# roboyu/Kimera-Multi

Measured on AMD Instinct MI355X. Metric: dpgo edges*iters/sec (+ LC candidates verified/sec in 'lcd'), higher is better.
Workload: dtype f64

## Files before the change

kimera-multi_amd/csrc/pgo.hip:

```cpp
#include <hip/hip_runtime.h>
#include <hip/hip_ext.h>
#include <rccl/rccl.h>
#include <dlfcn.h>

#include <algorithm>
#include <chrono>
#include <thread>
#include <cmath>
#include <cstdio>
#include <cstdlib>
#include <cstring>
#include <limits>
#include <numeric>
#include <string>
#include <vector>

#include "common.h"

#ifndef KMX_HESS_PROBE
#define KMX_HESS_PROBE 0
#endif

namespace {

constexpr int WAVES = 4;
constexpr int BLOCK = 64 * WAVES;
constexpr int NPART = 4;
constexpr int RED_BYTES = 8 * NPART * WAVES + 16;

enum Phase { PH_IDLE = 0, PH_START = 1, PH_TCG = 2, PH_STEP = 3 };
// ... 35 lines not shown
__device__ __forceinline__ Gnc load_gnc(const Gnc* p) {
  Gnc s;
  s.inner = p->inner; s.updates = p->updates; s.fired = p->fired; s.rounds = p->rounds;
  s.mu = p->mu; s.pad[0] = s.pad[1] = s.pad[2] = 0.0;
  return s;
}
__device__ __forceinline__ void store_gnc(Gnc* p, const Gnc& s) {
  p->inner = s.inner; p->updates = s.updates; p->fired = s.fired; p->rounds = s.rounds; p->mu = s.mu;
}

struct HostStatus {
  unsigned long long word;
};
__device__ __forceinline__ void post_status(HostStatus* hs, int l, unsigned long long seq, bool running) {
  __hip_atomic_store(&hs[l].word, (seq << 1) | (running ? 1ull : 0ull), __ATOMIC_RELAXED, __HIP_MEMORY_SCOPE_SYSTEM);
}

struct Params {
  int tcg_max, rtr_iters, use_precond, robust;
  double kappa, theta, Delta0, Delta_max, accept_rho, gn_tol, shift, barc, mu_step, rel_tol;
  int gnc_on, inner_iters, max_updates, n_ext;
  int rgd;
  double rgd_step;
  int early_stop;
};

struct alignas(16) TileDesc {
  int robot, p0, k0, np_n;
  int rt0, rt1;
  int pad0, pad1;
};

struct Dev {
  int ntiles, L, nloc, npub;
  int gt0, gnt;
  const TileDesc* tile;
  const int* rtile0;
  const int* inc_ptr;
  double* rec;
  const int* rec_o;
  double* ekappa;
  double* etau;
  double* ew;
  const int2* eipos;
  double *X, *Xt, *g, *r, *z, *hd, *S, *Pinv, *hD, *pub;
  double* hDS;
  double* dh;
// ... 61 lines not shown
  return s;
}

template <int R>
__device__ __forceinline__ double gsum(double x, int base) {
  double s = 0.0;
#pragma unroll
  for (int k = 0; k < R; ++k) s += __shfl(x, base + k, 64);
  return s;
}

__device__ __forceinline__ void load4(const double* p, double v[4]) {
  const double2* q = reinterpret_cast<const double2*>(p);
  double2 a = q[0], b = q[1];
  v[0] = a.x; v[1] = a.y; v[2] = b.x; v[3] = b.y;
}
__device__ __forceinline__ void store4(double* p, const double v[4]) {
  double2* q = reinterpret_cast<double2*>(p);
  q[0] = make_double2(v[0], v[1]);
  q[1] = make_double2(v[2], v[3]);
}

constexpr int SYM4 = 10;
__device__ __forceinline__ void load_sym4(const double* p, double M[16]) {
  const double2* p2 = reinterpret_cast<const double2*>(p);
  const double2 a = p2[0], b = p2[1], c = p2[2], e = p2[3], f = p2[4];
  M[0] = a.x; M[1] = M[4] = a.y; M[2] = M[8] = b.x; M[3] = M[12] = b.y;
  M[5] = c.x; M[6] = M[9] = c.y; M[7] = M[13] = e.x;
  M[10] = e.y; M[11] = M[14] = f.x;
  M[15] = f.y;
}
__device__ __forceinline__ void load_sym3(const double* p, double S[9]) {
  S[0] = p[0]; S[1] = S[3] = p[1]; S[2] = S[6] = p[2];
  S[4] = p[3]; S[5] = S[7] = p[4];
  S[8] = p[5];
}

__device__ __forceinline__ void lds_barrier() { asm volatile("s_waitcnt lgkmcnt(0)\n\ts_barrier" ::: "memory"); }

struct Edge {
  double R[9], t[3], wk, wt;
};

__device__ __forceinline__ int2 unpack_int2(double v) {
  const long long b = __double_as_longlong(v);
  return make_int2((int)(b & 0xffffffffll), (int)(b >> 32));
}

template <int RW>
struct Rec {
  static constexpr int Q = RW / 2;
  static constexpr int GS = RW == 10 ? 8 : 16;
  static constexpr int WK = RW == 10 ? 6 : 12;
  __device__ static __forceinline__ void load(const Dev& d, size_t k, double2 q[Q]) {
    if constexpr (RW == 10) {
      const double2* p2 = reinterpret_cast<const double2*>(d.rec + (size_t)GS * k);
      const double2 a0 = p2[0], a1 = p2[1], a2 = p2[2], a3 = p2[3];
      const unsigned raw = (unsigned)d.rec_o[k];
      const int other = (int)(raw << 3) >> 3;
      const unsigned big = raw >> 29;
      const double qa = a0.x, qb = a0.y, qc = a1.x;
      const double ql = sqrt(1.0 - (qa * qa + qb * qb + qc * qc));
      const double w = big == 0 ? ql : qa, x = big == 0 ? qa : (big == 1 ? ql : qb);
      const double y = big <= 1 ? qb : (big == 2 ? ql : qc), z = big == 3 ? ql : qc;
      q[0] = make_double2(w, x);
      q[1] = make_double2(y, z);
      q[2] = make_double2(a1.y, a2.x);
      q[3] = make_double2(a2.y, a3.x);
      const double wt = a3.y;
      const long long bits = (long long)(unsigned)other | (std::signbit(wt) ? (1ll << 63) : 0ll);
      q[4] = make_double2(std::fabs(wt), __longlong_as_double(bits));
    } else {
      const double2* q2 = reinterpret_cast<const double2*>(d.rec + (size_t)GS * k);
#pragma unroll
      for (int i = 0; i < Q; ++i) q[i] = q2[i];
    }
  }
  __device__ static __forceinline__ double wt_word(double wt, bool tail) {
    return (RW == 10 && tail) ? -wt : wt;
  }
  __device__ static __forceinline__ void edge(const double2 q[Q], Edge& E) {
    if constexpr (RW == 10) {
      const double w = q[0].x, x = q[0].y, y = q[1].x, z = q[1].y;
      const double xx = x * x, yy = y * y, zz = z * z, xy = x * y, xz = x * z, yz = y * z;
      const double wx = w * x, wy = w * y, wz = w * z;
      E.R[0] = 1.0 - 2.0 * (yy + zz); E.R[1] = 2.0 * (xy - wz); E.R[2] = 2.0 * (xz + wy);
      E.R[3] = 2.0 * (xy + wz); E.R[4] = 1.0 - 2.0 * (xx + zz); E.R[5] = 2.0 * (yz - wx);
      E.R[6] = 2.0 * (xz - wy); E.R[7] = 2.0 * (yz + wx); E.R[8] = 1.0 - 2.0 * (xx + yy);
      E.t[0] = q[2].x; E.t[1] = q[2].y; E.t[2] = q[3].x;
      E.wk = q[3].y;
      E.wt = q[4].x;
    } else {
      E.R[0] = q[0].x; E.R[1] = q[0].y; E.R[2] = q[1].x; E.R[3] = q[1].y; E.R[4] = q[2].x;
      E.R[5] = q[2].y; E.R[6] = q[3].x; E.R[7] = q[3].y; E.R[8] = q[4].x;
      E.t[0] = q[4].y; E.t[1] = q[5].x; E.t[2] = q[5].y;
      E.wk = q[6].x;
      E.wt = q[6].y;
    }
  }
// ... 191 lines not shown
  static constexpr int ptr_off = x_off + TP * R * 32;
  static constexpr int red_off = ptr_off + ((TP + 1) * 4 + 15) / 16 * 16;
  static constexpr int bytes = red_off + 8 * NPART * W + 16;
};
template <int R, int W = WAVES>
struct SmemC {
  static constexpr int TP = W * (64 / R);
  static constexpr int x_off = 0;
  static constexpr int ptr_off = TP * R * 32;
  static constexpr int red_off = ptr_off + ((TP + 1) * 4 + 15) / 16 * 16;
  static constexpr int bytes = red_off + 8 * NPART * W + 16;
};
constexpr int SCR_BYTES = BLOCK * 6 * 8;
struct SmemU {
  static constexpr int red_off = SCR_BYTES;
  static constexpr int bytes = red_off + RED_BYTES;
};
static_assert(SCR_BYTES <= SmemH<3>::ptr_off && SCR_BYTES <= SmemH<8>::ptr_off, "scratch");
static_assert(SCR_BYTES <= SmemHG<3>::x_off, "scratch");

struct NoPre {
  __device__ bool operator()() const { return true; }
};
template <int R, int RW, bool REC_FIRST, typename Src, typename Pre, bool DIAG = true, int W = WAVES>
__device__ __forceinline__ bool hinc_gather_src(const Dev& d, const Lane& L, Src& src, double acc[4], char* smem,
                                                Pre&& pre) {
  using SM = SmemH<R, W>;
  using RC = Rec<RW>;
  constexpr int CH = SM::CH;
  double* Cs = reinterpret_cast<double*>(smem + SM::c_off);
  int* sptr = reinterpret_cast<int*>(smem + SM::ptr_off);
  const int tid = threadIdx.x;
  const int p0 = L.p0, np = L.np, K0 = L.k0, n = L.n;
  const int pl = L.pose - p0;
  const int lt = min(tid, CH - 1);
  acc[0] = acc[1] = acc[2] = acc[3] = 0.0;
  auto ld = [&](int c0, double2* q) { RC::load(d, (size_t)(K0 + max(min(c0 + lt, n - 1), 0)), q); };
  double2 q[RC::Q];
  if constexpr (REC_FIRST) ld(0, q);
  if (tid <= np) sptr[tid] = d.inc_ptr[p0 + tid] - K0;
  if constexpr (!REC_FIRST) ld(0, q);
  __syncthreads();
  if (!pre()) return false;
  for (int c0 = 0; c0 < n; c0 += CH) {
    Edge E;
    RC::edge(q, E);
    const int2 in = RC::inc(q);
    const int o = in.x;
    const bool tail = (in.y >> 31) & 1;
    double2 vr[2 * R];
    src.nbr(o, vr);
    if (tid < CH && c0 + tid < n) {
      const double wk = (o >= 0) ? E.wk : 0.0, wt = (o >= 0) ? E.wt : 0.0;
#pragma unroll
      for (int a = 0; a < R; ++a) {
        const double v0 = vr[2 * a].x, v1 = vr[2 * a].y, v2 = vr[2 * a + 1].x, v3 = vr[2 * a + 1].y;
        double h[4];
        if (tail) {
#pragma unroll
          for (int c = 0; c < 3; ++c)
            h[c] = -(wk * (v0 * E.R[c * 3 + 0] + v1 * E.R[c * 3 + 1] + v2 * E.R[c * 3 + 2]) + wt * v3 * E.t[c]);
          h[3] = -(wt * v3);
        } else {
#pragma unroll
          for (int c = 0; c < 3; ++c) h[c] = -(wk * (v0 * E.R[0 * 3 + c] + v1 * E.R[1 * 3 + c] + v2 * E.R[2 * 3 + c]));
          h[3] = -(wt * (v3 + (v0 * E.t[0] + v1 * E.t[1] + v2 * E.t[2])));
        }
        store4(Cs + (tid * R + a) * 4, h);
      }
    }
    asm volatile("" ::: "memory");
    ld(c0 + CH, q);
    lds_barrier();
    if (L.valid) {
      const int j0 = max(sptr[pl], c0) - c0, j1 = min(sptr[pl + 1], c0 + CH) - c0;
#pragma unroll 4
      for (int j = j0; j < j1; ++j) {
        double h[4];
        load4(Cs + (j * R + L.a) * 4, h);
        acc[0] += h[0]; acc[1] += h[1]; acc[2] += h[2]; acc[3] += h[3];
      }
    }
    lds_barrier();
  }
  if (DIAG && L.valid) {
    double vs[4];
    double D[16];
    src.own(L.pose, L.a, vs);
#if KMX_HESS_PROBE & 2
    for (int c = 0; c < 16; ++c) D[c] = (c % 5 == 0) ? 1.0 : 0.0;
#else
    load_sym4(d.hD + SYM4 * (size_t)L.pose, D);
#endif
#pragma unroll
    for (int c = 0; c < 4; ++c)
      acc[c] += vs[0] * D[4 * c] + vs[1] * D[4 * c + 1] + vs[2] * D[4 * c + 2] + vs[3] * D[4 * c + 3];
  }
  return true;
}

template <int R>
struct PlainRows {
  const double* V;
  __device__ __forceinline__ void nbr(int o, double2 vr[2 * R]) const {
    const double2* b2 = reinterpret_cast<const double2*>(V + (size_t)max(o, 0) * 4 * R);
#if KMX_HESS_PROBE & 1
#pragma unroll
    for (int i = 0; i < 2 * R; ++i) vr[i] = make_double2(1e-3 * i, 1e-3);
    (void)b2;
#else
#pragma unroll
    for (int i = 0; i < 2 * R; ++i) vr[i] = b2[i];
#endif
  }
  __device__ __forceinline__ void own(int pose, int a, double vs[4]) {
#if KMX_HESS_PROBE & 2
    for (int c = 0; c < 4; ++c) vs[c] = 1e-3 * c;
#else
    load4(V + (size_t)pose * 4 * R + 4 * a, vs);
#endif
  }
};
template <int R, int RW, bool REC_FIRST = false, bool DIAG = true, typename Pre = NoPre>
__device__ __forceinline__ bool hinc_gather(const Dev& d, const Lane& L, const double* V, double acc[4],
                                            char* smem, Pre&& pre = Pre{}) {
  PlainRows<R> src{V};
  return hinc_gather_src<R, RW, REC_FIRST, PlainRows<R>, Pre&, DIAG, WAVES>(d, L, src, acc, smem, pre);
}

template <int R, int RW, int W = WAVES>
__device__ __forceinline__ void hinc_grad(const Dev& d, const Lane& L, const double* V, const double* pub,
                                          double acc[4], double* cost, char* smem) {
  using SM = SmemHG<R, W>;
  using RC = Rec<RW>;
  constexpr int CH = SM::CH;
  double* Cs = reinterpret_cast<double*>(smem + SM::c_off);
  double2* xs = reinterpret_cast<double2*>(smem + SM::x_off);
  int* sptr = reinterpret_cast<int*>(smem + SM::ptr_off);
  const int tid = threadIdx.x;
  const int p0 = L.p0, np = L.np, K0 = L.k0, n = L.n;
  const int pl = L.pose - p0;
  const int lt = min(tid, CH - 1);
  acc[0] = acc[1] = acc[2] = acc[3] = 0.0;
  double csum = 0.0;
  auto ld = [&](int c0, double2* q) { RC::load(d, (size_t)(K0 + max(min(c0 + lt, n - 1), 0)), q); };
  double2 q[RC::Q];
  ld(0, q);
  if (tid <= np) sptr[tid] = d.inc_ptr[p0 + tid] - K0;
  {
    const double2* v2 = reinterpret_cast<const double2*>(V + (size_t)p0 * 4 * R);
// ... 612 lines not shown
    }
    vals[0] = m;
    vals[1] = ch;
  }
  double* lds = reinterpret_cast<double*>(smem);
#pragma unroll
  for (int s = 0; s < 2; ++s) {
    const double w = wave_sum(vals[s]);
    if ((threadIdx.x & 63) == 0) lds[s * WAVES + (threadIdx.x >> 6)] = w;
  }
  __syncthreads();
  if (threadIdx.x == 0) {
#pragma unroll
    for (int s = 0; s < 2; ++s) {
      double t = 0.0;
#pragma unroll
      for (int w = 0; w < WAVES; ++w) t += lds[s * WAVES + w];
      d.part[(size_t)L.tile * NPART + 2 + s] = t;
    }
  }
}

template <int R, int RW, int RM>
__device__ __forceinline__ void body_hess(const Dev& d, int first_launch, int slot, HostStatus* hs,
                                          unsigned long long seq, char* smem) {
  const Lane L = lane_map<R>(d);
  int tcg_iter;
  double beta;
  double y[4] = {0, 0, 0, 0}, zs[4] = {0, 0, 0, 0}, H[4];
  const size_t o = (size_t)L.pose * 4 * R + 4 * L.a;
  if constexpr (RM == RM_CONSUMER) {
    __shared__ Ctl cs;
    __shared__ double rl[NPART * WAVES];
    const Ctl& c0 = d.ctl[L.l];
    const bool writer = L.tile == L.rt0;
    if (writer && threadIdx.x < (int)(sizeof(Ctl) / 8))
      reinterpret_cast<double*>(&cs)[threadIdx.x] = reinterpret_cast<const double*>(&c0)[threadIdx.x];
    const bool grad = (first_launch & 1) != 0;
    const bool upd = !grad;
    RobotSum<2> rs;
    RobotSum<3> rg;
    if (upd) rs.issue(d.part_u, 2, L.rt0, L.rt1);
    if (grad) rg.issue(d.part, NPART, L.rt0, L.rt1);
    const int ph0 = c0.phase;
    const bool active = ph0 == (grad ? PH_START : PH_TCG);
    auto idle = [&]() {
      if (writer && threadIdx.x == 0) {
        d.ctl2[L.l] = c0;
        if (hs) post_status(hs, L.l, seq, false);
      }
    };
    if (!active && (!d.p.early_stop || (first_launch & 2))) {
      idle();
      return;
    }
    UpdStep u{0, 0, 0.0};
    auto decide = [&]() {
      if (!active) {
        idle();
        return false;
      }
      double tot[NPART] = {0.0, 0.0, 0.0, 0.0};
      if (upd) rs.finish(d.part_u, 2, rl, tot);
      if (grad) rg.finish(d.part, NPART, rl, tot);
      if (upd) u = upd_step(c0.mode, c0.r_stop, c0.lin_stop, c0.z_r, c0.tcg_iter, tot[0], tot[1], d.p);
      if (grad) u.done = sqrt(tot[1]) < d.p.gn_tol ? 1 : 0;
      if (writer && threadIdx.x == 0) {
        if (upd || grad) control_on(cs, d, L.l, grad ? RED_GRAD : RED_UPDATE, tot, R, true);
        d.ctl2[L.l] = cs;
        if (hs) post_status(hs, L.l, seq, cs.phase == PH_TCG);
      }
      return !u.done;
    };
    bool go;
    if (d.p.early_stop) {
      go = hinc_gather<R, RW, false, false>(d, L, d.z, H, smem, decide);
    } else {
      hinc_gather<R, RW, false, false>(d, L, d.z, H, smem);
      go = decide();
    }
    if (!go) return;
    tcg_iter = grad ? 0 : c0.tcg_iter;
    beta = u.beta;
  } else {
    const Ctl& c = d.ctl[L.l];
    const int ph = c.phase;
    tcg_iter = c.tcg_iter;
    beta = c.beta;
    if ((first_launch & 2) && ph != PH_TCG) return;
    if (!hinc_gather<R, RW, true, false>(d, L, d.z, H, smem, [&]() { return ph == PH_TCG; })) return;
  }
  const bool first = (tcg_iter == 0) || (KMX_HESS_PROBE & 4);
  asm volatile("" ::: "memory");
  const int dhn = d.dhn;
  double dold[4] = {0, 0, 0, 0}, hold[4] = {0, 0, 0, 0};
  if (L.valid) {
    double Dg[16];
#if KMX_HESS_PROBE & 2
    for (int k = 0; k < 4; ++k) zs[k] = 1e-3 * k;
    for (int c = 0; c < 16; ++c) Dg[c] = (c % 5 == 0) ? 1.0 : 0.0;
#else
    load4(d.z + o, zs);
    load_sym4(d.hDS + SYM4 * (size_t)L.pose, Dg);
#endif
    if (!first) {
      load4(d.dh + (size_t)((tcg_iter - 1) % dhn) * d.vec + o, dold);
      load4(d.hd + o, hold);
    }
#pragma unroll
    for (int c = 0; c < 4; ++c)
      H[c] += zs[0] * Dg[4 * c] + zs[1] * Dg[4 * c + 1] + zs[2] * Dg[4 * c + 2] + zs[3] * Dg[4 * c + 3];
  }
  double hz[4];
#pragma unroll
  for (int k = 0; k < 4; ++k) hz[k] = H[k];
  (void)y;
  double v = 0.0;
  double dl[4] = {0, 0, 0, 0}, hdl[4] = {0, 0, 0, 0};
  if (L.valid) {
    if (first) {
#pragma unroll
      for (int k = 0; k < 4; ++k) { dl[k] = -zs[k]; hdl[k] = -hz[k]; }
    } else {
#pragma unroll
      for (int k = 0; k < 4; ++k) {
        dl[k] = -zs[k] + beta * dold[k];
        hdl[k] = -hz[k] + beta * hold[k];
      }
      if (tcg_iter >= dhn && tcg_iter % dhn == 0) {
        double et[4] = {0, 0, 0, 0};
        if (tcg_iter > dhn) load4(d.eta + o, et);
// ... 507 lines not shown
    if (threadIdx.x == 0 && writer) {
      control_on(cs, d, L.l, RED_COST, tot, R, true);
      cs.phase = PH_STEP;
      d.ctl[L.l] = cs;
    }
  } else {
    commit = d.ctl[L.l].commit != 0;
  }
  if (!commit || !L.valid) return;
  const size_t o = (size_t)L.pose * 4 * R + 4 * L.a;
  double v[4];
  load4(d.Xt + o, v);
  store4(d.X + o, v);
  if (!final) return;
  const int s = d.pose_slot[L.pose];
  if (s >= 0) store4(d.pub + (size_t)s * 4 * R + 4 * L.a, v);
}

template <int R, int RW, int RM>
__global__ __launch_bounds__(BLOCK, LB<R>::w) void k_grad(Dev d, int gated) {
  KMX_SMEM;
  body_grad<R, RW, RM>(d, gated, smem);
}
template <int R, int RW, int RM>
__global__ __launch_bounds__(BLOCK, LB<R>::w) void k_hess(Dev d, int first, int slot, HostStatus* hs,
                                                          unsigned long long seq) {
  KMX_SMEM;
  body_hess<R, RW, RM>(d, first, slot, hs, seq, smem);
}
template <int R, int RM>
__global__ __launch_bounds__(BLOCK) void k_update(Dev d, HostStatus* hs, unsigned long long seq, int slot) {
  KMX_SMEM;
  body_update<R, RM>(d, hs, seq, slot, smem);
}
template <int R, int RW>
__global__ __launch_bounds__(BLOCK, (R <= 5 ? 3 : 2)) void k_step(Dev d, const Ctl* cin, Ctl* cout, int jl, int slot,
                                                                  HostStatus* hs, unsigned long long seq) {
  KMX_SMEM;
  body_step<R, RW>(d, cin, cout, jl, slot, hs, seq, smem);
}
template <int R>
__global__ __launch_bounds__(BLOCK) void k_retract(Dev d, int fold, const Ctl* src) {
  KMX_SMEM;
  body_retract<R>(d, fold, src, smem);
}
template <int R, int RW, int RM>
__global__ __launch_bounds__(BLOCK, LB<R>::w) void k_cost(Dev d, const Ctl* src) {
  KMX_SMEM;
  body_cost<R, RW, RM>(d, src, smem);
}
template <int R>
// ... 456 lines not shown
  int *d_xs_rseg = nullptr, *d_xr_rseg = nullptr;
  double *d_xsbuf = nullptr, *d_xrbuf = nullptr;
  long long xn_send = 0, xn_recv = 0;
  std::vector<long long> xs_cnt, xr_cnt, xs_off, xr_off;
  int blind_left = 0;
  static constexpr int BLIND_SLACK = 2, BLIND_WINDOW = 8;
  static constexpr int MAX_GROUPS = 4;
  struct Group {
    int l0 = 0, l1 = 0;
    int t0 = 0, nt = 0;
    int blind_left = 0;
  };
  int groups_req = 2;
  std::vector<Group> grp;
  int grm = 2;
  int grm_forced = -1;
  static constexpr int GROUP_CONSUMER_MAX_TILES = 384;
  hipStream_t gstream[MAX_GROUPS - 1] = {nullptr, nullptr, nullptr};
  hipEvent_t ev_fork = nullptr, ev_join[MAX_GROUPS - 1] = {nullptr, nullptr, nullptr};
  bool hess_gate = true;
  int rm = RM_LAUNCH;
  int rm_forced = -1;
  int early_stop = 1;
  static constexpr int RM_CONSUMER_MAX_POSES = 80000;
  bool poll_timeout = false;
  bool timing = false;
  int* d_hv_launch = nullptr;
  std::vector<hipEvent_t> ev_pool;
  size_t ev_used = 0;
  double *d_accV = nullptr, *d_accY = nullptr;
  double acc_gamma = 0.0;
  int acc_k = 0;
  bool acc_ready = false, acc_started = false;
};

namespace {

void rot_to_quat(const double* R, double* q) {
  const double tr = R[0] + R[4] + R[8];
  double w, x, y, z;
  if (tr > 0.0) {
    const double s = 2.0 * std::sqrt(tr + 1.0);
    w = 0.25 * s; x = (R[7] - R[5]) / s; y = (R[2] - R[6]) / s; z = (R[3] - R[1]) / s;
  } else if (R[0] > R[4] && R[0] > R[8]) {
    const double s = 2.0 * std::sqrt(1.0 + R[0] - R[4] - R[8]);
    w = (R[7] - R[5]) / s; x = 0.25 * s; y = (R[1] + R[3]) / s; z = (R[2] + R[6]) / s;
// ... 119 lines not shown

void sync_params(kmx_pgo* h) {
  Params& p = h->dv.p;
  p.tcg_max = h->P.tcg_max_iterations;
  p.rtr_iters = h->P.rtr_iterations;
  p.use_precond = h->P.use_preconditioner;
  p.robust = h->P.robust_cost == KMX_COST_GNC_TLS ? 1 : 0;
  p.kappa = h->P.tcg_kappa;
  p.theta = h->P.tcg_theta;
  p.Delta0 = h->P.rtr_initial_radius;
  p.Delta_max = h->P.rtr_max_radius;
  p.accept_rho = h->P.rtr_accept_rho;
  p.gn_tol = h->P.gradnorm_tol;
  p.shift = h->P.precond_shift;
  p.barc = h->P.gnc_barc;
  p.mu_step = h->P.gnc_mu_step;
  p.rel_tol = h->gnc_rel_tol;
  p.gnc_on = h->gnc_on;
  p.inner_iters = h->gnc_inner_iters;
  p.max_updates = h->gnc_max_updates;
  p.n_ext = h->n_ext;
  p.rgd = h->P.method == KMX_METHOD_RGD ? 1 : 0;
  p.rgd_step = h->P.rgd_stepsize;
  p.early_stop = h->early_stop;
  h->dv.ext = h->d_ext;
}

void enqueue_publish(kmx_pgo* h) {
  const int ps = 4 * h->P.r;
  const long long tot = h->n_owned * ps;
  if (tot == 0) return;
  hipLaunchKernelGGL(k_publish, dim3((unsigned)((tot / 2 + 255) / 256)), dim3(256), 0, h->stream, h->d_vec,
                     h->d_pub + (size_t)h->first_owned * ps, h->d_pub_src + h->first_owned, (int)h->n_owned, ps);
}

template <int RW>
void enqueue_precond_t(kmx_pgo* h, int gated) {
  const int blocks = std::max(1, std::min(gated ? 256 : 1024, (h->nloc + 127) / 128));
  hipLaunchKernelGGL(k_precond<RW>, dim3(blocks), dim3(128), 0, h->stream, h->dv, gated);
}
void enqueue_precond(kmx_pgo* h, int gated) {
  if (h->rw == 10) enqueue_precond_t<10>(h, gated);
  else enqueue_precond_t<16>(h, gated);
}

bool enqueue_begin(kmx_pgo* h, const unsigned char* d_active, int mode, bool defer = false,
                   hipEvent_t done = nullptr) {
// ... 61 lines not shown
void red_g(const GroupLaunch& q, int kind, HostStatus* hs = nullptr, unsigned long long seq = 0,
           hipEvent_t done = nullptr) {
  if (done)
    hipExtLaunchKernelGGL(k_reduce, dim3(q.nl), dim3(RBLOCK), 0, q.s, nullptr, done, 0u, q.d, q.l0, kind, R, hs, seq, -1,
                          (const double*)nullptr);
  else
    hipLaunchKernelGGL(k_reduce, dim3(q.nl), dim3(RBLOCK), 0, q.s, q.d, q.l0, kind, R, hs, seq, -1,
                       (const double*)nullptr);
}

template <int RM>
bool fold_grad(const kmx_pgo* h) {
  return RM == RM_CONSUMER && h->P.method != KMX_METHOD_RGD && h->P.tcg_max_iterations > 0;
}
template <int RM>
bool fold_cost(const kmx_pgo* h) {
  return RM == RM_CONSUMER && (h->P.rtr_iterations == 1 || h->P.method == KMX_METHOD_RGD);
}

template <int R, int RW, int RM>
void enqueue_grad_t(kmx_pgo* h, int gated = 0) {
  hipLaunchKernelGGL((k_grad<R, RW, RM>), dim3(h->ntiles), dim3(BLOCK), SmemHG<R>::bytes, h->stream, h->dv, gated);
  if (!fold_grad<RM>(h)) red_t<R, RM>(h, RED_GRAD);
}

template <int R, int RW, int RM>
void enqueue_tcg_t(kmx_pgo* h) {
  const dim3 grid(h->ntiles), blk(BLOCK);
  unsigned long long prev = 0;
  bool poll = h->poll && h->hstat;
  if (poll && h->poll_auto && h->blind_left > 0) {
    --h->blind_left;
    poll = false;
  }
  const int tmax = h->P.tcg_max_iterations;
  int steps = tmax;
  h->tcg_stopped = false;
  if constexpr (RM == RM_CONSUMER) {
    if (onesync(h)) {
      int J = tmax + 1;
      for (int j = 0; j <= tmax; ++j) {
        hipEvent_t e0 = nullptr, e1 = nullptr;
        int slot = -1;
        if (h->timing && h->ev_used / 2 < (size_t)HV_SLOTS) {
          slot = (int)(h->ev_used / 2);
          e0 = next_event(h);
// ... 15 lines not shown
          break;
        }
      }
      h->ctl_par = J & 1;
      steps = J - 1;
      if (poll && h->poll_auto && steps + kmx_pgo::BLIND_SLACK >= tmax) h->blind_left = kmx_pgo::BLIND_WINDOW;
      return;
    }
  }
  for (int j = 0; j < tmax; ++j) {
    hipEvent_t e0 = nullptr, e1 = nullptr;
    int slot = -1;
    if (h->timing && h->ev_used / 2 < (size_t)HV_SLOTS) {
      slot = (int)(h->ev_used / 2);
      e0 = next_event(h);
      e1 = next_event(h);
    }
    poll = poll && h->poll;
    const unsigned long long seq = poll ? ++h->seq : 0;
    HostStatus* hs = poll ? h->hstat : nullptr;
    const bool gate = j > 0 && h->hess_gate;
    const int fl = (j == 0 ? 1 : 0) | (gate ? 2 : 0);
    if constexpr (RM == RM_CONSUMER) {
      if (slot >= 0)
        hipExtLaunchKernelGGL((k_hess<R, RW, RM>), grid, blk, SmemH<R>::bytes, h->stream, e0, e1, 0u, h->dv,
                              fl, slot, hs, seq);
      else
        hipLaunchKernelGGL((k_hess<R, RW, RM>), grid, blk, SmemH<R>::bytes, h->stream, h->dv, fl, slot,
                           hs, seq);
      hipLaunchKernelGGL((k_update<R, RM>), grid, blk, SmemU::bytes, h->stream, h->dv, nullptr, 0ull, slot);
      if (poll && j > 0 && !wait_running(h, seq, 0, h->dv.L)) {
        steps = j + 1;
        h->tcg_stopped = true;
        break;
      }
      continue;
    }
    if (slot >= 0)
      hipExtLaunchKernelGGL((k_hess<R, RW, RM>), grid, blk, SmemH<R>::bytes, h->stream, e0, e1, 0u, h->dv, fl, slot,
                            (HostStatus*)nullptr, 0ull);
    else
      hipLaunchKernelGGL((k_hess<R, RW, RM>), grid, blk, SmemH<R>::bytes, h->stream, h->dv, fl, slot, nullptr, 0ull);
    red_t<R, RM>(h, RED_HESS, nullptr, 0, slot);
    hipLaunchKernelGGL((k_update<R, RM>), grid, blk, SmemU::bytes, h->stream, h->dv, nullptr, seq, -1);
    red_t<R, RM>(h, RED_UPDATE, hs, seq, -1, nullptr);
    if (poll) {
      if (j > 0 && !wait_running(h, prev, 0, h->dv.L)) {
        steps = j + 1;
        break;
      }
      prev = seq;
    }
  }
  if (poll && h->poll_auto && steps + kmx_pgo::BLIND_SLACK >= tmax) h->blind_left = kmx_pgo::BLIND_WINDOW;
}

template <int R, int RW, int RM>
void enqueue_trial_t(kmx_pgo* h, bool rgd) {
  const dim3 grid(h->ntiles), blk(BLOCK);
  const bool os = RM == RM_CONSUMER && !rgd && onesync(h);
  const Ctl* src = os && h->ctl_par ? h->d_ctl2 : h->d_ctl;
  const bool cons = RM == RM_CONSUMER && !rgd;
  if (!os && !(cons && h->tcg_stopped))
    hipLaunchKernelGGL((k_retract<R>), grid, blk, SmemU::bytes, h->stream, h->dv, cons ? 2 : 0, (const Ctl*)h->d_ctl);
  hipLaunchKernelGGL((k_cost<R, RW, RM>), grid, blk, SmemC<R>::bytes, h->stream, h->dv, src);
// ... 22 lines not shown
    int steps[kmx_pgo::MAX_GROUPS];
    for (int g = 0; g < G; ++g) {
      poll[g] = h->poll && h->hstat;
      if (poll[g] && h->poll_auto && h->grp[g].blind_left > 0) {
        --h->grp[g].blind_left;
        poll[g] = false;
      }
      live[g] = true;
      stopped[g] = false;
      prev[g] = seq[g] = 0;
      steps[g] = tmax;
    }
    for (int j = 0; j < tmax; ++j) {
      bool any = false;
      for (int g = 0; g < G; ++g) {
        if (!live[g]) continue;
        any = true;
        poll[g] = poll[g] && h->poll;
        seq[g] = poll[g] ? ++h->seq : 0;
        HostStatus* hs = poll[g] ? h->hstat : nullptr;
        const int fl = (j == 0 ? 1 : 0) | (j > 0 && h->hess_gate ? 2 : 0);
        const dim3 grid(q[g].d.gnt);
        if constexpr (cons) {
          hipLaunchKernelGGL((k_hess<R, RW, RM>), grid, blk, SmemH<R>::bytes, q[g].s, q[g].d, fl, -1, hs, seq[g]);
          hipLaunchKernelGGL((k_update<R, RM>), grid, blk, SmemU::bytes, q[g].s, q[g].d, (HostStatus*)nullptr, 0ull,
                             -1);
        } else {
          hipLaunchKernelGGL((k_hess<R, RW, RM>), grid, blk, SmemH<R>::bytes, q[g].s, q[g].d, fl, -1,
                             (HostStatus*)nullptr, 0ull);
          red_g<R>(q[g], RED_HESS);
          hipLaunchKernelGGL((k_update<R, RM>), grid, blk, SmemU::bytes, q[g].s, q[g].d, (HostStatus*)nullptr,
                             seq[g], -1);
          red_g<R>(q[g], RED_UPDATE, hs, seq[g]);
        }
      }
      if (!any) break;
      for (int g = 0; g < G; ++g) {
        if (!live[g] || !poll[g]) continue;
        if (j > 0 && !wait_running(h, cons ? seq[g] : prev[g], h->grp[g].l0, h->grp[g].l1)) {
          steps[g] = j + 1;
          live[g] = false;
          stopped[g] = true;
        }
        prev[g] = seq[g];
      }
    }
    for (int g = 0; g < G; ++g)
      if (poll[g] && h->poll_auto && steps[g] + kmx_pgo::BLIND_SLACK >= tmax)
        h->grp[g].blind_left = kmx_pgo::BLIND_WINDOW;
    for (int g = 0; g < G; ++g) {
      const dim3 grid(q[g].d.gnt);
      const bool last = it + 1 == iters;
// ... 125 lines not shown
  KMX_CHECK(params->method == KMX_METHOD_RTR || params->method == KMX_METHOD_RGD, KMX_EUNSUP,
            "method must be KMX_METHOD_RTR or KMX_METHOD_RGD");
  KMX_CHECK(params->tcg_form == KMX_TCG_FORM_STANDARD || params->tcg_form == KMX_TCG_FORM_ONESYNC, KMX_EINVAL,
            "tcg_form must be KMX_TCG_FORM_STANDARD or KMX_TCG_FORM_ONESYNC");
  KMX_CHECK(params->method != KMX_METHOD_RGD || params->rgd_stepsize > 0.0, KMX_EINVAL, "rgd_stepsize must be > 0");
  KMX_CHECK(params->tile_incidences >= 0, KMX_EINVAL, "tile_incidences must be >= 0 (0: automatic)");
  int ndev = 0;
  KMX_HIP(hipGetDeviceCount(&ndev));
  KMX_CHECK(device >= 0 && device < ndev, KMX_EINVAL, "bad HIP device ordinal");
  KMX_HIP(hipSetDevice(device));
  kmx_pgo* h = new kmx_pgo();
  h->P = *params;
  h->device = device;
  hipError_t e = hipStreamCreateWithFlags(&h->stream, hipStreamNonBlocking);
  if (e != hipSuccess) {
    delete h;
    return kmx::fail(KMX_EHIP, std::string("hipStreamCreate: ") + hipGetErrorString(e));
  }
  h->own_stream = true;
  if (const char* v = std::getenv("KMX_RED")) {
    const int m = std::atoi(v);
    h->rm_forced = m == 0 ? RM_LAUNCH : m == 2 ? RM_CONSUMER : -1;
  }
  if (const char* v = std::getenv("KMX_HESS_GATE")) h->hess_gate = std::atoi(v) != 0;
  if (const char* v = std::getenv("KMX_TCG_GROUPS")) {
    const int g = std::atoi(v);
    h->groups_req = g >= 4 ? 4 : g >= 2 ? 2 : 1;
  }
  if (const char* v = std::getenv("KMX_GROUP_RED")) h->grm_forced = std::atoi(v) == 2 ? RM_CONSUMER : RM_LAUNCH;
  for (int g = 1; g < h->groups_req && e == hipSuccess; ++g) {
    e = hipStreamCreateWithFlags(&h->gstream[g - 1], hipStreamNonBlocking);
    if (e == hipSuccess) e = hipEventCreate(&h->ev_join[g - 1]);
  }
  if (e == hipSuccess && h->groups_req > 1) e = hipEventCreate(&h->ev_fork);
  if (e != hipSuccess) {
    (void)kmx_pgo_destroy(h);
    return kmx::fail(KMX_EHIP, std::string("robot group streams: ") + hipGetErrorString(e));
  }
  *out = h;
  return KMX_OK;
  KMX_GUARD_END
}

extern "C" int kmx_pgo_destroy(kmx_pgo* h) {
  if (!h) return KMX_OK;
  (void)hipSetDevice(h->device);
// ... 68 lines not shown
  KMX_HIP(hipStreamSynchronize(h->stream));
  free_dev(h);
  free_xchg(h);
  accel_reset(h);
  const int r = h->P.r, ps = 4 * r;
  h->n_robots = n_robots;
  h->npose.assign(n_poses, n_poses + n_robots);
  h->local_of.assign(n_robots, -1);
  h->robots.clear();
  h->loff.clear();
  int nloc = 0;
  for (int a = 0; a < n_robots; ++a) {
    KMX_CHECK(n_poses[a] >= 0, KMX_EINVAL, "negative pose count");
    if (local[a]) {
      h->local_of[a] = (int)h->robots.size();
      h->robots.push_back(a);
      h->loff.push_back(nloc);
      nloc += n_poses[a];
    }
  }
  h->nloc = nloc;
  h->rm = h->rm_forced >= 0 ? h->rm_forced : (nloc <= kmx_pgo::RM_CONSUMER_MAX_POSES ? RM_CONSUMER : RM_LAUNCH);
  if (onesync(h)) h->rm = RM_CONSUMER;
  h->early_stop = nloc <= kmx_pgo::RM_CONSUMER_MAX_POSES ? 1 : 0;
  const int L = (int)h->robots.size();
  KMX_CHECK(L > 0, KMX_EINVAL, "no local robot");
  KMX_CHECK(L <= 1024, KMX_EUNSUP, "at most 1024 local robots per handle");
  h->m_global = m;
  std::vector<int64_t> keys;
  for (int64_t e = 0; e < m; ++e) {
    KMX_CHECK(r1[e] >= 0 && r1[e] < n_robots && r2[e] >= 0 && r2[e] < n_robots, KMX_EINVAL,
              "edge robot id out of range");
    KMX_CHECK(p1[e] >= 0 && p1[e] < n_poses[r1[e]] && p2[e] >= 0 && p2[e] < n_poses[r2[e]], KMX_EINVAL,
              "edge pose id out of range");
    KMX_CHECK(!(r1[e] == r2[e] && p1[e] == p2[e]), KMX_EINVAL, "self-loop edge");
    if (r1[e] != r2[e]) {
      keys.push_back(((int64_t)r1[e] << 32) | (uint32_t)p1[e]);
      keys.push_back(((int64_t)r2[e] << 32) | (uint32_t)p2[e]);
    }
  }
  std::sort(keys.begin(), keys.end());
  keys.erase(std::unique(keys.begin(), keys.end()), keys.end());
  h->pub_key = keys;
  h->npub = (int64_t)keys.size();
  auto slot_of = [&](int rb, int pp) -> int64_t {
    const int64_t k = ((int64_t)rb << 32) | (uint32_t)pp;
    auto it = std::lower_bound(h->pub_key.begin(), h->pub_key.end(), k);
// ... 1069 lines not shown
```

Before: 972.8 million.

## Prefetch neighbour rows and epilogue loads in Hessian gather, specialize kernel per mode

Splits compact record loading into a stored part and an incidence word so the gather can prefetch the next chunk's neighbour rows and incidence word one iteration ahead. Adds an epilogue hook that issues the diagonal-block, z and previous-direction loads during the last chunk so they overlap the final reduction. It also turns the runtime grad/early-stop flags into template parameters with four kernel instantiations chosen on the host. The cost is more live registers from the prefetched rows and more compiled kernel variants.

```diff
diff --git a/kimera-multi_amd/csrc/pgo.hip b/kimera-multi_amd/csrc/pgo.hip
--- a/kimera-multi_amd/csrc/pgo.hip
+++ b/kimera-multi_amd/csrc/pgo.hip
@@ -6,6 +6,7 @@
 #include <algorithm>
 #include <chrono>
 #include <thread>
+#include <type_traits>
 #include <cmath>
 #include <cstdio>
 #include <cstdlib>
@@ -87,7 +88,6 @@
   int gnc_on, inner_iters, max_updates, n_ext;
   int rgd;
   double rgd_step;
-  int early_stop;
 };
 
 struct alignas(16) TileDesc {
@@ -195,14 +195,18 @@
 }
 
 constexpr int SYM4 = 10;
-__device__ __forceinline__ void load_sym4(const double* p, double M[16]) {
-  const double2* p2 = reinterpret_cast<const double2*>(p);
+__device__ __forceinline__ void expand_sym4(const double2 p2[5], double M[16]) {
   const double2 a = p2[0], b = p2[1], c = p2[2], e = p2[3], f = p2[4];
   M[0] = a.x; M[1] = M[4] = a.y; M[2] = M[8] = b.x; M[3] = M[12] = b.y;
   M[5] = c.x; M[6] = M[9] = c.y; M[7] = M[13] = e.x;
   M[10] = e.y; M[11] = M[14] = f.x;
   M[15] = f.y;
 }
+__device__ __forceinline__ void load_sym4(const double* p, double M[16]) {
+  const double2* p2 = reinterpret_cast<const double2*>(p);
+  const double2 v[5] = {p2[0], p2[1], p2[2], p2[3], p2[4]};
+  expand_sym4(v, M);
+}
 __device__ __forceinline__ void load_sym3(const double* p, double S[9]) {
   S[0] = p[0]; S[1] = S[3] = p[1]; S[2] = S[6] = p[2];
   S[4] = p[3]; S[5] = S[7] = p[4];
@@ -225,11 +229,23 @@
   static constexpr int Q = RW / 2;
   static constexpr int GS = RW == 10 ? 8 : 16;
   static constexpr int WK = RW == 10 ? 6 : 12;
-  __device__ static __forceinline__ void load(const Dev& d, size_t k, double2 q[Q]) {
+  static constexpr int QS = RW == 10 ? 4 : Q;
+  __device__ static __forceinline__ void load_stored(const Dev& d, size_t k, double2 a[QS]) {
+    const double2* p2 = reinterpret_cast<const double2*>(d.rec + (size_t)GS * k);
+#pragma unroll
+    for (int i = 0; i < QS; ++i) a[i] = p2[i];
+  }
+  __device__ static __forceinline__ unsigned load_word(const Dev& d, size_t k) {
+    static_assert(RW == 10, "compact records only");
+    return (unsigned)d.rec_o[k];
+  }
+  __device__ static __forceinline__ int other_of(unsigned word) {
+    static_assert(RW == 10, "compact records only");
+    return (int)(word << 3) >> 3;
+  }
+  __device__ static __forceinline__ void expand(const double2 a[QS], unsigned raw, double2 q[Q]) {
     if constexpr (RW == 10) {
-      const double2* p2 = reinterpret_cast<const double2*>(d.rec + (size_t)GS * k);
-      const double2 a0 = p2[0], a1 = p2[1], a2 = p2[2], a3 = p2[3];
-      const unsigned raw = (unsigned)d.rec_o[k];
+      const double2 a0 = a[0], a1 = a[1], a2 = a[2], a3 = a[3];
       const int other = (int)(raw << 3) >> 3;
       const unsigned big = raw >> 29;
       const double qa = a0.x, qb = a0.y, qc = a1.x;
@@ -244,10 +260,16 @@
       const long long bits = (long long)(unsigned)other | (std::signbit(wt) ? (1ll << 63) : 0ll);
       q[4] = make_double2(std::fabs(wt), __longlong_as_double(bits));
     } else {
-      const double2* q2 = reinterpret_cast<const double2*>(d.rec + (size_t)GS * k);
-#pragma unroll
-      for (int i = 0; i < Q; ++i) q[i] = q2[i];
-    }
+#pragma unroll
+      for (int i = 0; i < Q; ++i) q[i] = a[i];
+    }
+  }
+  __device__ static __forceinline__ void load(const Dev& d, size_t k, double2 q[Q]) {
+    double2 a[QS];
+    load_stored(d, k, a);
+    unsigned word = 0;
+    if constexpr (RW == 10) word = load_word(d, k);
+    expand(a, word, q);
   }
   __device__ static __forceinline__ double wt_word(double wt, bool tail) {
     return (RW == 10 && tail) ? -wt : wt;
@@ -485,9 +507,14 @@
 struct NoPre {
   __device__ bool operator()() const { return true; }
 };
-template <int R, int RW, bool REC_FIRST, typename Src, typename Pre, bool DIAG = true, int W = WAVES>
+struct NoEpi {
+  __device__ void operator()() const {}
+};
+template <int R, int RW, bool REC_FIRST, typename Src, typename Pre, bool DIAG = true, int W = WAVES,
+          bool PF = false, typename Epi = NoEpi>
 __device__ __forceinline__ bool hinc_gather_src(const Dev& d, const Lane& L, Src& src, double acc[4], char* smem,
-                                                Pre&& pre) {
+                                                Pre&& pre, Epi&& epi = Epi{}) {
+  static_assert(!PF || RW == 10, "the row prefetch reads rec_o ahead: compact records only");
   using SM = SmemH<R, W>;
   using RC = Rec<RW>;
   constexpr int CH = SM::CH;
@@ -498,21 +525,36 @@
   const int pl = L.pose - p0;
   const int lt = min(tid, CH - 1);
   acc[0] = acc[1] = acc[2] = acc[3] = 0.0;
-  auto ld = [&](int c0, double2* q) { RC::load(d, (size_t)(K0 + max(min(c0 + lt, n - 1), 0)), q); };
-  double2 q[RC::Q];
-  if constexpr (REC_FIRST) ld(0, q);
+  auto at = [&](int c0) { return (size_t)(K0 + max(min(c0 + lt, n - 1), 0)); };
+  double2 qs[RC::QS];
+  unsigned wo = 0, wo_next = 0;
+  auto ld = [&](int c0) {
+    RC::load_stored(d, at(c0), qs);
+    if constexpr (RW == 10 && !PF) wo = RC::load_word(d, at(c0));
+  };
+  if constexpr (REC_FIRST) ld(0);
   if (tid <= np) sptr[tid] = d.inc_ptr[p0 + tid] - K0;
-  if constexpr (!REC_FIRST) ld(0, q);
+  if constexpr (!REC_FIRST) ld(0);
+  if constexpr (PF) {
+    wo = RC::load_word(d, at(0));
+    wo_next = RC::load_word(d, at(CH));
+  }
   __syncthreads();
   if (!pre()) return false;
-  for (int c0 = 0; c0 < n; c0 += CH) {
+  double2 vr[2 * R];
+  if constexpr (PF) {
+    if (n > 0) src.nbr(RC::other_of(wo), vr);
+  }
+  auto chunk = [&](const int c0, auto last_c) __attribute__((always_inline)) {
+    constexpr bool LAST = decltype(last_c)::value;
+    double2 q[RC::Q];
+    RC::expand(qs, wo, q);
     Edge E;
     RC::edge(q, E);
     const int2 in = RC::inc(q);
     const int o = in.x;
     const bool tail = (in.y >> 31) & 1;
-    double2 vr[2 * R];
-    src.nbr(o, vr);
+    if constexpr (!PF) src.nbr(o, vr);
     if (tid < CH && c0 + tid < n) {
       const double wk = (o >= 0) ? E.wk : 0.0, wt = (o >= 0) ? E.wt : 0.0;
 #pragma unroll
@@ -533,7 +575,16 @@
       }
     }
     asm volatile("" ::: "memory");
-    ld(c0 + CH, q);
+    if constexpr (LAST) {
+      epi();
+    } else {
+      ld(c0 + CH);
+      if constexpr (PF) {
+        wo = wo_next;
+        src.nbr(RC::other_of(wo), vr);
+        wo_next = RC::load_word(d, at(c0 + 2 * CH));
+      }
+    }
     lds_barrier();
     if (L.valid) {
       const int j0 = max(sptr[pl], c0) - c0, j1 = min(sptr[pl + 1], c0 + CH) - c0;
@@ -545,6 +596,14 @@
       }
     }
     lds_barrier();
+  };
+  if constexpr (PF || !std::is_same_v<std::decay_t<Epi>, NoEpi>) {
+    int c0 = 0;
+    for (; c0 + CH < n; c0 += CH) chunk(c0, std::false_type{});
+    if (n > 0) chunk(c0, std::true_type{});
+    else epi();
+  } else {
+    for (int c0 = 0; c0 < n; c0 += CH) chunk(c0, std::false_type{});
   }
   if (DIAG && L.valid) {
     double vs[4];
@@ -584,11 +643,12 @@
 #endif
   }
 };
-template <int R, int RW, bool REC_FIRST = false, bool DIAG = true, typename Pre = NoPre>
+template <int R, int RW, bool REC_FIRST = false, bool DIAG = true, bool PF = false, typename Pre = NoPre,
+          typename Epi = NoEpi>
 __device__ __forceinline__ bool hinc_gather(const Dev& d, const Lane& L, const double* V, double acc[4],
-                                            char* smem, Pre&& pre = Pre{}) {
+                                            char* smem, Pre&& pre = Pre{}, Epi&& epi = Epi{}) {
   PlainRows<R> src{V};
-  return hinc_gather_src<R, RW, REC_FIRST, PlainRows<R>, Pre&, DIAG, WAVES>(d, L, src, acc, smem, pre);
+  return hinc_gather_src<R, RW, REC_FIRST, PlainRows<R>, Pre&, DIAG, WAVES, PF, Epi&>(d, L, src, acc, smem, pre, epi);
 }
 
 template <int R, int RW, int W = WAVES>
@@ -1247,13 +1307,39 @@
 }
 
 template <int R, int RW, int RM>
-__device__ __forceinline__ void body_hess(const Dev& d, int first_launch, int slot, HostStatus* hs,
+struct HessPF {
+  static constexpr bool rows = RW == 10 && (R >= 5 || RM == RM_CONSUMER);
+};
+template <int R, int RW, int RM, bool GRAD, bool EARLY>
+__device__ __forceinline__ void body_hess(const Dev& d, int gated, int slot, HostStatus* hs,
                                           unsigned long long seq, char* smem) {
+  static_assert(RM == RM_CONSUMER || (!GRAD && !EARLY), "the launched form has one body");
   const Lane L = lane_map<R>(d);
   int tcg_iter;
   double beta;
   double y[4] = {0, 0, 0, 0}, zs[4] = {0, 0, 0, 0}, H[4];
   const size_t o = (size_t)L.pose * 4 * R + 4 * L.a;
+  const int dhn = d.dhn;
+  double dold[4] = {0, 0, 0, 0}, hold[4] = {0, 0, 0, 0};
+  double2 dg[5];
+  bool first;
+  auto epi = [&]() {
+    if (L.valid) {
+#if KMX_HESS_PROBE & 2
+      for (int k = 0; k < 4; ++k) zs[k] = 1e-3 * k;
+      for (int c = 0; c < 5; ++c) dg[c] = make_double2(c == 0 || c == 2 ? 1.0 : 0.0, c >= 3 ? 1.0 : 0.0);
+#else
+      load4(d.z + o, zs);
+      const double2* p2 = reinterpret_cast<const double2*>(d.hDS + SYM4 * (size_t)L.pose);
+#pragma unroll
+      for (int c = 0; c < 5; ++c) dg[c] = p2[c];
+#endif
+      if (!first) {
+        load4(d.dh + (size_t)((tcg_iter - 1) % dhn) * d.vec + o, dold);
+        load4(d.hd + o, hold);
+      }
+    }
+  };
   if constexpr (RM == RM_CONSUMER) {
     __shared__ Ctl cs;
     __shared__ double rl[NPART * WAVES];
@@ -1261,24 +1347,25 @@
     const bool writer = L.tile == L.rt0;
     if (writer && threadIdx.x < (int)(sizeof(Ctl) / 8))
       reinterpret_cast<double*>(&cs)[threadIdx.x] = reinterpret_cast<const double*>(&c0)[threadIdx.x];
-    const bool grad = (first_launch & 1) != 0;
-    const bool upd = !grad;
-    RobotSum<2> rs;
-    RobotSum<3> rg;
-    if (upd) rs.issue(d.part_u, 2, L.rt0, L.rt1);
-    if (grad) rg.issue(d.part, NPART, L.rt0, L.rt1);
+    using RS = std::conditional_t<GRAD, RobotSum<3>, RobotSum<2>>;
+    const double* const part = GRAD ? d.part : d.part_u;
+    constexpr int stride = GRAD ? NPART : 2;
+    RS rs;
+    if constexpr (EARLY) rs.issue(part, stride, L.rt0, L.rt1);
     const int ph0 = c0.phase;
-    const bool active = ph0 == (grad ? PH_START : PH_TCG);
+    const bool active = ph0 == (GRAD ? PH_START : PH_TCG);
     auto idle = [&]() {
       if (writer && threadIdx.x == 0) {
         d.ctl2[L.l] = c0;
         if (hs) post_status(hs, L.l, seq, false);
       }
     };
-    if (!active && (!d.p.early_stop || (first_launch & 2))) {
+    if (!active && (!EARLY || gated)) {
       idle();
       return;
     }
+    tcg_iter = GRAD ? 0 : c0.tcg_iter;
+    first = (tcg_iter == 0) || (KMX_HESS_PROBE & 4);
     UpdStep u{0, 0, 0.0};
     auto decide = [&]() {
       if (!active) {
@@ -1286,52 +1373,43 @@
         return false;
       }
       double tot[NPART] = {0.0, 0.0, 0.0, 0.0};
-      if (upd) rs.finish(d.part_u, 2, rl, tot);
-      if (grad) rg.finish(d.part, NPART, rl, tot);
-      if (upd) u = upd_step(c0.mode, c0.r_stop, c0.lin_stop, c0.z_r, c0.tcg_iter, tot[0], tot[1], d.p);
-      if (grad) u.done = sqrt(tot[1]) < d.p.gn_tol ? 1 : 0;
+      rs.finish(part, stride, rl, tot);
+      if constexpr (GRAD) u.done = sqrt(tot[1]) < d.p.gn_tol ? 1 : 0;
+      else u = upd_step(c0.mode, c0.r_stop, c0.lin_stop, c0.z_r, c0.tcg_iter, tot[0], tot[1], d.p);
       if (writer && threadIdx.x == 0) {
-        if (upd || grad) control_on(cs, d, L.l, grad ? RED_GRAD : RED_UPDATE, tot, R, true);
+        control_on(cs, d, L.l, GRAD ? RED_GRAD : RED_UPDATE, tot, R, true);
         d.ctl2[L.l] = cs;
         if (hs) post_status(hs, L.l, seq, cs.phase == PH_TCG);
       }
       return !u.done;
     };
     bool go;
-    if (d.p.early_stop) {
-      go = hinc_gather<R, RW, false, false>(d, L, d.z, H, smem, decide);
+    if constexpr (EARLY) {
+      go = hinc_gather<R, RW, false, false, HessPF<R, RW, RM>::rows>(d, L, d.z, H, smem, decide, epi);
     } else {
-      hinc_gather<R, RW, false, false>(d, L, d.z, H, smem);
+      auto epi_late = [&]() {
+        epi();
+        rs.issue(part, stride, L.rt0, L.rt1);
+      };
+      hinc_gather<R, RW, false, false, HessPF<R, RW, RM>::rows>(d, L, d.z, H, smem, NoPre{}, epi_late);
       go = decide();
     }
     if (!go) return;
-    tcg_iter = grad ? 0 : c0.tcg_iter;
     beta = u.beta;
   } else {
     const Ctl& c = d.ctl[L.l];
     const int ph = c.phase;
     tcg_iter = c.tcg_iter;
     beta = c.beta;
-    if ((first_launch & 2) && ph != PH_TCG) return;
-    if (!hinc_gather<R, RW, true, false>(d, L, d.z, H, smem, [&]() { return ph == PH_TCG; })) return;
-  }
-  const bool first = (tcg_iter == 0) || (KMX_HESS_PROBE & 4);
-  asm volatile("" ::: "memory");
-  const int dhn = d.dhn;
-  double dold[4] = {0, 0, 0, 0}, hold[4] = {0, 0, 0, 0};
+    first = (tcg_iter == 0) || (KMX_HESS_PROBE & 4);
+    if (gated && ph != PH_TCG) return;
+    if (!hinc_gather<R, RW, true, false, HessPF<R, RW, RM>::rows>(d, L, d.z, H, smem,
+                                                                  [&]() { return ph == PH_TCG; }, epi))
+      return;
+  }
   if (L.valid) {
     double Dg[16];
-#if KMX_HESS_PROBE & 2
-    for (int k = 0; k < 4; ++k) zs[k] = 1e-3 * k;
-    for (int c = 0; c < 16; ++c) Dg[c] = (c % 5 == 0) ? 1.0 : 0.0;
-#else
-    load4(d.z + o, zs);
-    load_sym4(d.hDS + SYM4 * (size_t)L.pose, Dg);
-#endif
-    if (!first) {
-      load4(d.dh + (size_t)((tcg_iter - 1) % dhn) * d.vec + o, dold);
-      load4(d.hd + o, hold);
-    }
+    expand_sym4(dg, Dg);
 #pragma unroll
     for (int c = 0; c < 4; ++c)
       H[c] += zs[0] * Dg[4 * c] + zs[1] * Dg[4 * c + 1] + zs[2] * Dg[4 * c + 2] + zs[3] * Dg[4 * c + 3];
@@ -1885,11 +1963,11 @@
   KMX_SMEM;
   body_grad<R, RW, RM>(d, gated, smem);
 }
-template <int R, int RW, int RM>
-__global__ __launch_bounds__(BLOCK, LB<R>::w) void k_hess(Dev d, int first, int slot, HostStatus* hs,
+template <int R, int RW, int RM, bool GRAD, bool EARLY>
+__global__ __launch_bounds__(BLOCK, LB<R>::w) void k_hess(Dev d, int gated, int slot, HostStatus* hs,
                                                           unsigned long long seq) {
   KMX_SMEM;
-  body_hess<R, RW, RM>(d, first, slot, hs, seq, smem);
+  body_hess<R, RW, RM, GRAD, EARLY>(d, gated, slot, hs, seq, smem);
 }
 template <int R, int RM>
 __global__ __launch_bounds__(BLOCK) void k_update(Dev d, HostStatus* hs, unsigned long long seq, int slot) {
@@ -2392,6 +2470,7 @@
   int rm = RM_LAUNCH;
   int rm_forced = -1;
   int early_stop = 1;
+  int decide_forced = -1;
   static constexpr int RM_CONSUMER_MAX_POSES = 80000;
   bool poll_timeout = false;
   bool timing = false;
@@ -2557,7 +2636,6 @@
   p.n_ext = h->n_ext;
   p.rgd = h->P.method == KMX_METHOD_RGD ? 1 : 0;
   p.rgd_step = h->P.rgd_stepsize;
-  p.early_stop = h->early_stop;
   h->dv.ext = h->d_ext;
 }
 
@@ -2665,6 +2743,28 @@
 void enqueue_grad_t(kmx_pgo* h, int gated = 0) {
   hipLaunchKernelGGL((k_grad<R, RW, RM>), dim3(h->ntiles), dim3(BLOCK), SmemHG<R>::bytes, h->stream, h->dv, gated);
   if (!fold_grad<RM>(h)) red_t<R, RM>(h, RED_GRAD);
+}
+
+template <int R, int RW, int RM>
+void launch_hess(const kmx_pgo* h, dim3 grid, hipStream_t st, const Dev& dv, int fl, int slot, HostStatus* hs,
+                 unsigned long long seq, hipEvent_t e0 = nullptr, hipEvent_t e1 = nullptr) {
+  const dim3 blk(BLOCK);
+  const int gated = (fl & 2) ? 1 : 0;
+  auto go = [&](auto kern) {
+    if (e0)
+      hipExtLaunchKernelGGL(kern, grid, blk, SmemH<R>::bytes, st, e0, e1, 0u, dv, gated, slot, hs, seq);
+    else
+      hipLaunchKernelGGL(kern, grid, blk, SmemH<R>::bytes, st, dv, gated, slot, hs, seq);
+  };
+  if constexpr (RM == RM_CONSUMER) {
+    const bool grad = (fl & 1) != 0, early = h->early_stop != 0;
+    if (grad && early) go(k_hess<R, RW, RM, true, true>);
+    else if (grad) go(k_hess<R, RW, RM, true, false>);
+    else if (early) go(k_hess<R, RW, RM, false, true>);
+    else go(k_hess<R, RW, RM, false, false>);
+  } else {
+    go(k_hess<R, RW, RM, false, false>);
+  }
 }
 
 template <int R, int RW, int RM>
@@ -2726,12 +2826,7 @@
     const bool gate = j > 0 && h->hess_gate;
     const int fl = (j == 0 ? 1 : 0) | (gate ? 2 : 0);
     if constexpr (RM == RM_CONSUMER) {
-      if (slot >= 0)
-        hipExtLaunchKernelGGL((k_hess<R, RW, RM>), grid, blk, SmemH<R>::bytes, h->stream, e0, e1, 0u, h->dv,
-                              fl, slot, hs, seq);
-      else
-        hipLaunchKernelGGL((k_hess<R, RW, RM>), grid, blk, SmemH<R>::bytes, h->stream, h->dv, fl, slot,
-                           hs, seq);
+      launch_hess<R, RW, RM>(h, grid, h->stream, h->dv, fl, slot, hs, seq, e0, e1);
       hipLaunchKernelGGL((k_update<R, RM>), grid, blk, SmemU::bytes, h->stream, h->dv, nullptr, 0ull, slot);
       if (poll && j > 0 && !wait_running(h, seq, 0, h->dv.L)) {
         steps = j + 1;
@@ -2740,11 +2835,7 @@
       }
       continue;
     }
-    if (slot >= 0)
-      hipExtLaunchKernelGGL((k_hess<R, RW, RM>), grid, blk, SmemH<R>::bytes, h->stream, e0, e1, 0u, h->dv, fl, slot,
-                            (HostStatus*)nullptr, 0ull);
-    else
-      hipLaunchKernelGGL((k_hess<R, RW, RM>), grid, blk, SmemH<R>::bytes, h->stream, h->dv, fl, slot, nullptr, 0ull);
+    launch_hess<R, RW, RM>(h, grid, h->stream, h->dv, fl, slot, nullptr, 0ull, e0, e1);
     red_t<R, RM>(h, RED_HESS, nullptr, 0, slot);
     hipLaunchKernelGGL((k_update<R, RM>), grid, blk, SmemU::bytes, h->stream, h->dv, nullptr, seq, -1);
     red_t<R, RM>(h, RED_UPDATE, hs, seq, -1, nullptr);
@@ -2813,12 +2904,11 @@
         const int fl = (j == 0 ? 1 : 0) | (j > 0 && h->hess_gate ? 2 : 0);
         const dim3 grid(q[g].d.gnt);
         if constexpr (cons) {
-          hipLaunchKernelGGL((k_hess<R, RW, RM>), grid, blk, SmemH<R>::bytes, q[g].s, q[g].d, fl, -1, hs, seq[g]);
+          launch_hess<R, RW, RM>(h, grid, q[g].s, q[g].d, fl, -1, hs, seq[g]);
           hipLaunchKernelGGL((k_update<R, RM>), grid, blk, SmemU::bytes, q[g].s, q[g].d, (HostStatus*)nullptr, 0ull,
                              -1);
         } else {
-          hipLaunchKernelGGL((k_hess<R, RW, RM>), grid, blk, SmemH<R>::bytes, q[g].s, q[g].d, fl, -1,
-                             (HostStatus*)nullptr, 0ull);
+          launch_hess<R, RW, RM>(h, grid, q[g].s, q[g].d, fl, -1, nullptr, 0ull);
           red_g<R>(q[g], RED_HESS);
           hipLaunchKernelGGL((k_update<R, RM>), grid, blk, SmemU::bytes, q[g].s, q[g].d, (HostStatus*)nullptr,
                              seq[g], -1);
@@ -2990,6 +3080,7 @@
     const int m = std::atoi(v);
     h->rm_forced = m == 0 ? RM_LAUNCH : m == 2 ? RM_CONSUMER : -1;
   }
+  if (const char* v = std::getenv("KMX_HESS_DECIDE")) h->decide_forced = std::atoi(v) != 0 ? 1 : 0;
   if (const char* v = std::getenv("KMX_HESS_GATE")) h->hess_gate = std::atoi(v) != 0;
   if (const char* v = std::getenv("KMX_TCG_GROUPS")) {
     const int g = std::atoi(v);
@@ -3104,7 +3195,7 @@
   h->nloc = nloc;
   h->rm = h->rm_forced >= 0 ? h->rm_forced : (nloc <= kmx_pgo::RM_CONSUMER_MAX_POSES ? RM_CONSUMER : RM_LAUNCH);
   if (onesync(h)) h->rm = RM_CONSUMER;
-  h->early_stop = nloc <= kmx_pgo::RM_CONSUMER_MAX_POSES ? 1 : 0;
+  h->early_stop = h->decide_forced >= 0 ? h->decide_forced : (nloc <= kmx_pgo::RM_CONSUMER_MAX_POSES ? 1 : 0);
   const int L = (int)h->robots.size();
   KMX_CHECK(L > 0, KMX_EINVAL, "no local robot");
   KMX_CHECK(L <= 1024, KMX_EUNSUP, "at most 1024 local robots per handle");
```

Result: faster. 1.022 billion, median of 6 (+5.0%).
